# aclyde11/molecular-VAE

Measured on AMD Instinct MI355X. Metric: molecules/s (ELBO fwd+bwd+step), higher is better.
Workload: dtype bf16

## Files before the change

### molecular-vae_amd/csrc/rnn.hip

```cpp
#include "tile_pipe.hpp"
#include "kernels.hpp"
#include <stdlib.h>

template <typename T> __device__ __forceinline__ void load8(const T* p, float (&v)[8]);
template <> __device__ __forceinline__ void load8<float>(const float* p, float (&v)[8]) {
  const float4 a = *reinterpret_cast<const float4*>(p), b = *reinterpret_cast<const float4*>(p + 4);
  v[0] = a.x; v[1] = a.y; v[2] = a.z; v[3] = a.w; v[4] = b.x; v[5] = b.y; v[6] = b.z; v[7] = b.w;
}
template <> __device__ __forceinline__ void load8<bf16_t>(const bf16_t* p, float (&v)[8]) {
  const uint4 u = *reinterpret_cast<const uint4*>(p);
  const uint32_t w[4] = {u.x, u.y, u.z, u.w};
#pragma unroll
  for (int i = 0; i < 4; ++i) { v[2 * i] = __builtin_bit_cast(float, w[i] << 16); v[2 * i + 1] = __builtin_bit_cast(float, w[i] & 0xffff0000u); }
}
template <typename T> __device__ __forceinline__ void store8(T* p, const float (&v)[8]);
template <> __device__ __forceinline__ void store8<float>(float* p, const float (&v)[8]) {
  *reinterpret_cast<float4*>(p) = make_float4(v[0], v[1], v[2], v[3]);
  *reinterpret_cast<float4*>(p + 4) = make_float4(v[4], v[5], v[6], v[7]);
}
template <> __device__ __forceinline__ void store8<bf16_t>(bf16_t* p, const float (&v)[8]) {
  uint4 u;
  u.x = (uint32_t)f2bf(v[0]) | ((uint32_t)f2bf(v[1]) << 16); u.y = (uint32_t)f2bf(v[2]) | ((uint32_t)f2bf(v[3]) << 16);
  u.z = (uint32_t)f2bf(v[4]) | ((uint32_t)f2bf(v[5]) << 16); u.w = (uint32_t)f2bf(v[6]) | ((uint32_t)f2bf(v[7]) << 16);
  *reinterpret_cast<uint4*>(p) = u;
}
template <typename T> __device__ __forceinline__ void ldn(const T* p, float (&v)[8], int n, bool vec) {
  if (vec && n == 8) { load8<T>(p, v); return; }
#pragma unroll
  for (int e = 0; e < 8; ++e) v[e] = (e < n) ? TT<T>::ld(p + e) : 0.f;
}
template <typename T> __device__ __forceinline__ void stn(T* p, const float (&v)[8], int n, bool vec) {
  if (vec && n == 8) { store8<T>(p, v); return; }
#pragma unroll
  for (int e = 0; e < 8; ++e) if (e < n) TT<T>::st(p + e, v[e]);
}

template <typename T> __device__ __forceinline__ float act_sigmoid(float x);
template <typename T> __device__ __forceinline__ float act_tanh(float x);
template <> __device__ __forceinline__ float act_sigmoid<float>(float x) { return 1.f / (1.f + expf(-x)); }
template <> __device__ __forceinline__ float act_tanh<float>(float x) { return tanhf(x); }
template <> __device__ __forceinline__ float act_sigmoid<bf16_t>(float x) { return __builtin_amdgcn_rcpf(1.f + __expf(-x)); }
template <> __device__ __forceinline__ float act_tanh<bf16_t>(float x) { return fmaf(-2.f, __builtin_amdgcn_rcpf(1.f + __expf(2.f * x)), 1.f); }

__device__ __forceinline__ int xcd_remap_r(int bid, int n) {
  const int q = n >> 3, r = n & 7, x = bid & 7, i = bid >> 3;
  return (x < r ? x * (q + 1) : r * (q + 1) + (x - r) * q) + i;
}

struct DropArgs { float scale; uint32_t thresh, seed; };
__host__ __device__ __forceinline__ uint32_t drop_hash(uint32_t seed, uint32_t idx) {
  uint32_t h = idx * 0x9E3779B1u ^ seed;
  h ^= h >> 16; h *= 0x85EBCA6Bu; h ^= h >> 13; h *= 0xC2B2AE35u; h ^= h >> 16;
  return h;
}
__device__ __forceinline__ float drop_factor(const DropArgs& da, const uint8_t* mask, uint32_t idx0, long off) {
  const bool keep = mask ? (mask[off] != 0) : (drop_hash(da.seed, idx0 + (uint32_t)off) >= da.thresh);
  return keep ? da.scale : 0.f;
}

struct StepTaskF {
  const void *A0, *A1, *W0, *W1;
  long lda0, lda1, ldw0, ldw1;
  int K0, K1;
  const float* add; long add_ld;
  const float* add_tbl;
  const int64_t* add_idx; long add_idx_ld; int add_rows;
  const float* bias;
  const float* c_prev; float* c_out;
  void* c_save;
  void* h_out; long ldh;
  void* g_out;
  const void* hprev_t0;
  int t;
  void* h_drop;
  const uint8_t* dmask;
  uint32_t didx0;
};
struct StepArgsF { StepTaskF t[MVAE_MAX_LAYERS]; const int* lengths; int ntask, B, H, tiles_m, tiles_j, dbg, vec, cell, gru3; DropArgs drop; };

template <typename T, int BM, int BJ, int NBUF, bool WS = false>
__global__ __launch_bounds__(WS ? 512 : 256) void lstm_step_fwd_kernel(StepArgsF p) {
  constexpr bool PIPE = NBUF > 0;
  constexpr int NTHR = WS ? 512 : 256;
  static_assert(!WS || NBUF > 0, "wave specialisation needs the LDS-direct ring");
  extern __shared__ __attribute__((aligned(16))) char smem[];
  static_assert(BJ == 32 || BJ == 64, "hidden units per tile");
  constexpr int JS = BJ / 32;
  constexpr int BN = 4 * BJ, WM = BM / 2, MI = WM / 16, NI = 4 * JS;
  const int tid = threadIdx.x, lane = tid & 63, wave = (tid >> 6) & 3, wm = wave >> 1, wj = wave & 1;
  const int per_task = p.tiles_m * p.tiles_j;
  const int bid = xcd_remap_r(blockIdx.x, p.ntask * per_task);
  const int task = bid / per_task;
  const int rem = bid - task * per_task;
  const int tj = rem / p.tiles_m, tm = rem - tj * p.tiles_m;
  const StepTaskF& q = p.t[task];
  const int m0 = tm * BM, j0 = tj * BJ, H = p.H, B = p.B;

  f32x4 acc[MI][NI];
#pragma unroll
  for (int i = 0; i < MI; ++i)
#pragma unroll
    for (int g = 0; g < NI; ++g) acc[i][g] = f32x4{0.f, 0.f, 0.f, 0.f};

#ifdef MVAE_TUNING
  const bool run_main = !(p.dbg & 2);
#else
  constexpr bool run_main = true;
#endif
  if (run_main) {
  if constexpr (PIPE) {
    PipeSeg<BM, BN> s0, s1;
    const uint32_t sz = (uint32_t)sizeof(T);
    const int skip0 = p.gru3 ? 3 : -1, skip1 = p.gru3 ? 2 : -1;
    {
      const uint32_t lda = (uint32_t)q.lda0 * sz, ldw = (uint32_t)q.ldw0 * sz;
      auto offA = [&](int r) -> uint32_t { const int gm = m0 + r; return gm < B ? (uint32_t)gm * lda : PIPE_OOB; };
      auto offB = [&](int r) -> uint32_t { const int g = r / BJ, j = j0 + (r - g * BJ); return (j < H && g != skip0) ? (uint32_t)(g * H + j) * ldw : PIPE_OOB; };
      pipe_seg_init<T, BM, BN>(s0, q.A0, (uint32_t)B * lda, q.W0, (uint32_t)(4 * H) * ldw, offA, offB, q.K0, tid & 255);
    }
    {
      const uint32_t lda = (uint32_t)q.lda1 * sz, ldw = (uint32_t)q.ldw1 * sz;
      auto offA = [&](int r) -> uint32_t { const int gm = m0 + r; return gm < B ? (uint32_t)gm * lda : PIPE_OOB; };
      auto offB = [&](int r) -> uint32_t { const int g = r / BJ, j = j0 + (r - g * BJ); return (j < H && g != skip1) ? (uint32_t)(g * H + j) * ldw : PIPE_OOB; };
      pipe_seg_init<T, BM, BN>(s1, q.A1, (uint32_t)B * lda, q.W1, (uint32_t)(4 * H) * ldw, offA, offB, q.K1, tid & 255);
    }
    if constexpr (WS) tile_gemm_ws<T, BM, BN, MI, NI, (NBUF > 0 ? NBUF : 3), JS, BJ>(smem, s0, s1, wm * WM, wj * (BJ / 2), acc, tid);
    else tile_gemm_pipe<T, BM, BN, MI, NI, (NBUF > 0 ? NBUF : 3), JS, BJ>(smem, s0, s1, wm * WM, wj * (BJ / 2), acc, tid);
  } else {
    int brow[NI];
#pragma unroll
    for (int g = 0; g < NI; ++g) brow[g] = (g / JS) * BJ + wj * (BJ / 2) + (g % JS) * 16;
    if (q.A0 != nullptr) {
      const T* A = reinterpret_cast<const T*>(q.A0);
      const T* W = reinterpret_cast<const T*>(q.W0);
      const long lda = q.lda0, ldw = q.ldw0;
      auto rowA = [&](int r) -> const T* { const int gm = m0 + r; return gm < B ? A + (long)gm * lda : nullptr; };
      auto rowB = [&](int r) -> const T* { const int g = r / BJ, j = j0 + (r - g * BJ); return (j < H && !(p.gru3 && g == 3)) ? W + ((long)g * H + j) * ldw : nullptr; };
      tile_gemm_segment<T, BM, BN, MI, NI>(smem, rowA, rowB, 0, q.K0, wm * WM, brow, acc, tid);
    }
    if (q.A1 != nullptr) {
      const T* A = reinterpret_cast<const T*>(q.A1);
      const T* W = reinterpret_cast<const T*>(q.W1);
      const long lda = q.lda1, ldw = q.ldw1;
      auto rowA = [&](int r) -> const T* { const int gm = m0 + r; return gm < B ? A + (long)gm * lda : nullptr; };
      auto rowB = [&](int r) -> const T* { const int g = r / BJ, j = j0 + (r - g * BJ); return (j < H && !(p.gru3 && g == 2)) ? W + ((long)g * H + j) * ldw : nullptr; };
      tile_gemm_segment<T, BM, BN, MI, NI>(smem, rowA, rowB, 0, q.K1, wm * WM, brow, acc, tid);
    }
// ... 130 lines not shown
        c[e] = gf[e] * cp[e] + gi[e] * gg[e];
        h[e] = go[e] * act_tanh<T>(c[e]);
      }
      st32(q.c_out + (long)row * H + j8, c);
      stT(hout + (long)row * q.ldh + j8, h);
      if (q.h_drop) {
        float hd[8];
#pragma unroll
        for (int e = 0; e < 8; ++e) hd[e] = (e < n) ? h[e] * drop_factor(p.drop, q.dmask, q.didx0, (long)row * H + j8 + e) : 0.f;
        stT(reinterpret_cast<T*>(q.h_drop) + (long)row * q.ldh + j8, hd);
      }
      if (gout) {
        stT(csave + (long)row * H + j8, c);
        stT(g4, gi); stT(g4 + H, gf); stT(g4 + 2 * H, gg); stT(g4 + 3 * H, go);
      }
    } else {
      const bool valid = p.lengths ? (q.t < p.lengths[row]) : true;
      float gr[8], gz[8], gn[8], hs_[8], hseq[8];
#pragma unroll
      for (int e = 0; e < 8; ++e) {
        gr[e] = act_sigmoid<T>(pre[0][e]); gz[e] = act_sigmoid<T>(pre[1][e]);
        gn[e] = act_tanh<T>(pre[2][e] + gr[e] * pre[3][e]);
        const float hn = (1.f - gz[e]) * gn[e] + gz[e] * cp[e];
        hs_[e] = valid ? hn : cp[e];
        hseq[e] = valid ? hn : 0.f;
      }
      st32(q.c_out + (long)row * H + j8, hs_);
      stT(hout + (long)row * q.ldh + j8, hseq);
      if (q.h_drop) {
        float hd[8];
#pragma unroll
        for (int e = 0; e < 8; ++e) hd[e] = (e < n) ? hseq[e] * drop_factor(p.drop, q.dmask, q.didx0, (long)row * H + j8 + e) : 0.f;
        stT(reinterpret_cast<T*>(q.h_drop) + (long)row * q.ldh + j8, hd);
      }
      if (gout) { stT(g4, gr); stT(g4 + H, gz); stT(g4 + 2 * H, gn); stT(g4 + 3 * H, pre[3]); }
    }
  }
  };
  const bool has_add = q.add != nullptr || q.add_tbl != nullptr;
  if (fast) { if (has_add) rows(std::true_type{}, std::true_type{}); else rows(std::true_type{}, std::false_type{}); }
  else { if (has_add) rows(std::false_type{}, std::true_type{}); else rows(std::false_type{}, std::false_type{}); }
}

template <int BMW, int BNB, int NBUF, bool WS = false>
__global__ __launch_bounds__(WS ? 512 : BMW * 2) void lstm_step_fwd_gm_kernel(StepArgsF p) {
  using T = bf16_t;
  extern __shared__ __attribute__((aligned(16))) char smem[];
  static_assert(BMW == 256 || BMW == 128, "weight rows per tile: 64 or 32 units x 4 gates");
  static_assert(!WS || BMW == 128, "loader / consumer split: the 4-wave tile only");
  constexpr int NT = BMW * 2;
  constexpr int BU = BMW / 4;
  constexpr int MI = 8, NI = BNB / 64;
  const int tid = threadIdx.x, lane = tid & 63, wave = WS ? ((tid >> 6) & 3) : (tid >> 6), wm = wave >> 2, wn = wave & 3;
  const int per_task = p.tiles_m * p.tiles_j;
  const int bid = xcd_remap_r(blockIdx.x, p.ntask * per_task);
  const int task = bid / per_task;
  const int rem = bid - task * per_task;
  const int tj = rem / p.tiles_m, tm = rem - tj * p.tiles_m;
  const StepTaskF& q = p.t[task];
  const int n0 = tm * BNB, j0 = tj * BU, H = p.H, B = p.B;

  const int lq = lane >> 4, lc = lane & 15;
  const int ub = j0 + 32 * wm + 8 * lq;
  constexpr bool BIAS_FIRST = (BMW == 256 && BNB == 256);
  auto load_bias = [&](float (&bias)[4][8]) {
    if (q.bias) {
#pragma unroll
      for (int g = 0; g < 4; ++g) load8<float>(q.bias + g * H + ub, bias[g]);
    } else {
#pragma unroll
      for (int g = 0; g < 4; ++g)
#pragma unroll
        for (int e = 0; e < 8; ++e) bias[g][e] = 0.f;
    }
  };
  f32x4 acc[MI][NI];
  if constexpr (BIAS_FIRST) {
    float bias[4][8];
    load_bias(bias);
#pragma unroll
    for (int ni = 0; ni < NI; ++ni)
#pragma unroll
      for (int g = 0; g < 4; ++g)
#pragma unroll
        for (int e = 0; e < 8; ++e) acc[2 * g + (e >> 2)][ni][e & 3] = bias[g][e];
  } else {
#pragma unroll
    for (int i = 0; i < MI; ++i)
#pragma unroll
      for (int g = 0; g < NI; ++g) acc[i][g] = f32x4{0.f, 0.f, 0.f, 0.f};
  }

  float cpa[NI][8];
  auto load_cprev_all = [&]() {
    const float* cpsrc = q.c_prev ? q.c_prev : q.c_out;
#pragma unroll
    for (int ni = 0; ni < NI; ++ni) {
      const int row = n0 + wn * (16 * NI) + ni * 16 + lc;
      load8<float>(cpsrc + (long)(row < B ? row : B - 1) * H + ub, cpa[ni]);
    }
  };
  if constexpr (BIAS_FIRST) load_cprev_all();

#ifdef MVAE_TUNING
  const bool run_main = !(p.dbg & 2);
#else
  constexpr bool run_main = true;
#endif
  if (run_main) {
    PipeSeg<BMW, BNB, NT> s0, s1;
    auto wrow = [&](int r) -> int {
// ... 53 lines not shown
    if constexpr (decltype(has_add)::value) {
#pragma unroll
      for (int g = 0; g < 4; ++g) {
        float a[8];
        load8<float>(q.add + (long)row * q.add_ld + g * H + ub, a);
#pragma unroll
        for (int e = 0; e < 8; ++e) pre[g][e] += a[e];
      }
    }
    float gi[8], gf[8], gg[8], go[8], c[8], h[8];
#pragma unroll
    for (int e = 0; e < 8; ++e) {
      gi[e] = act_sigmoid<T>(pre[0][e]); gf[e] = act_sigmoid<T>(pre[1][e]); gg[e] = act_tanh<T>(pre[2][e]); go[e] = act_sigmoid<T>(pre[3][e]);
      c[e] = gf[e] * cp[e] + gi[e] * gg[e];
      h[e] = go[e] * act_tanh<T>(c[e]);
    }
#ifdef MVAE_TUNING
    const int srow = (p.dbg & 4) ? n0 + (row & 15) : row;
    const bool sgate = !(p.dbg & 8);
#else
    const int srow = row;
    constexpr bool sgate = true;
#endif
    store8<float>(q.c_out + (long)srow * H + ub, c);
    store8<T>(hout + (long)srow * q.ldh + ub, h);
    if (gout) {
      T* g4 = gout + (long)srow * 4 * H + ub;
      store8<T>(csave + (long)srow * H + ub, c);
      if (sgate) { store8<T>(g4, gi); store8<T>(g4 + H, gf); store8<T>(g4 + 2 * H, gg); store8<T>(g4 + 3 * H, go); }
    }
  }
  };
  const bool full = n0 + BNB <= B;
  if (q.add) { if (full) epilogue(std::true_type{}, std::true_type{}); else epilogue(std::true_type{}, std::false_type{}); }
  else { if (full) epilogue(std::false_type{}, std::true_type{}); else epilogue(std::false_type{}, std::false_type{}); }
}

struct StepTaskB {
  const void *A0, *A1, *W0, *W1;
  long lda0, lda1, ldw0, ldw1;
  int K0, K1;
  const float* dy; long dy_ld;
  const void* gates; const void* c; const void* c_prev;
  const float* dc_in; float* dc_out;
  void* dG; long ldg;
  const void* h_prev; long ldhp;
  float* dh0;
  int t;
  int seg1_full;
  int drop;
  const uint8_t* dmask;
  uint32_t didx0;
};
struct StepArgsB { StepTaskB t[MVAE_MAX_LAYERS]; const int* lengths; float* partial; int ntask, B, H, tiles_m, tiles_n, dbg, vec, cell, split, gru3; DropArgs drop; };

template <typename T>
__device__ __forceinline__ void bwd_cell_group(const StepArgsB& p, const StepTaskB& q, int row, int j8, int n, bool vec, float (&dh)[8]) {
  const int H = p.H;
  const T* gates = reinterpret_cast<const T*>(q.gates);
  const T* cs = reinterpret_cast<const T*>(q.c);
  const T* csp = reinterpret_cast<const T*>(q.c_prev);
  T* dG = reinterpret_cast<T*>(q.dG);
  const long o = (long)row * H + j8;
  float dci[8];
  if (q.dc_in) ldn<float>(q.dc_in + o, dci, n, vec);
  else {
#pragma unroll
    for (int e = 0; e < 8; ++e) dci[e] = 0.f;
  }
  if (p.cell == MVAE_CELL_LSTM) {
    if (q.dy) {
      float a[8];
      ldn<float>(q.dy + (long)row * q.dy_ld + j8, a, n, vec);
#pragma unroll
      for (int e = 0; e < 8; ++e) dh[e] += a[e];
    }
    float gi[8], gf[8], gg[8], go[8], c[8], cp[8];
    const T* g4 = gates + (long)row * 4 * H + j8;
    ldn<T>(g4, gi, n, vec); ldn<T>(g4 + H, gf, n, vec); ldn<T>(g4 + 2 * H, gg, n, vec); ldn<T>(g4 + 3 * H, go, n, vec);
    ldn<T>(cs + o, c, n, vec);
    if (csp) ldn<T>(csp + o, cp, n, vec);
    else {
#pragma unroll
      for (int e = 0; e < 8; ++e) cp[e] = 0.f;
    }
    float di[8], df[8], dg[8], dO[8], dco[8];
#pragma unroll
    for (int e = 0; e < 8; ++e) {
      const float tc = act_tanh<T>(c[e]);
      const float d_o = dh[e] * tc;
      const float dc = dh[e] * go[e] * (1.f - tc * tc) + dci[e];
      dco[e] = dc * gf[e];
      di[e] = dc * gg[e] * gi[e] * (1.f - gi[e]);
      df[e] = dc * cp[e] * gf[e] * (1.f - gf[e]);
      dg[e] = dc * gi[e] * (1.f - gg[e] * gg[e]);
      dO[e] = d_o * go[e] * (1.f - go[e]);
    }
    stn<float>(q.dc_out + o, dco, n, vec);
    T* d4 = dG + (long)row * q.ldg + j8;
    stn<T>(d4, di, n, vec); stn<T>(d4 + H, df, n, vec); stn<T>(d4 + 2 * H, dg, n, vec); stn<T>(d4 + 3 * H, dO, n, vec);
  } else {
#pragma unroll
    for (int e = 0; e < 8; ++e) dh[e] += dci[e];
    if (q.gates == nullptr) {
      stn<float>(q.dh0 + o, dh, n, vec);
      return;
    }
// ... 138 lines not shown
template <bool HAS_DY>
__device__ __forceinline__ void bwd_raw_load(const StepArgsB& p, const StepTaskB& q, int row, int j8, BwdRaw& r) {
  const int H = p.H;
  const bf16_t* gates = reinterpret_cast<const bf16_t*>(q.gates);
  const long o = (long)row * H + j8;
  const float* dsrc = (q.dc_in ? q.dc_in : q.dc_out) + o;
  r.dci[0] = *reinterpret_cast<const float4*>(dsrc); r.dci[1] = *reinterpret_cast<const float4*>(dsrc + 4);
  if (gates == nullptr) return;
  if constexpr (HAS_DY) {
    const float* ysrc = q.dy ? q.dy + (long)row * q.dy_ld + j8 : q.dc_out + o;
    r.dy[0] = *reinterpret_cast<const float4*>(ysrc); r.dy[1] = *reinterpret_cast<const float4*>(ysrc + 4);
  }
  const bf16_t* g4 = gates + (long)row * 4 * H + j8;
  r.g[0] = *reinterpret_cast<const uint4*>(g4); r.g[1] = *reinterpret_cast<const uint4*>(g4 + H);
  r.g[2] = *reinterpret_cast<const uint4*>(g4 + 2 * H); r.g[3] = *reinterpret_cast<const uint4*>(g4 + 3 * H);
  if (p.cell == MVAE_CELL_LSTM) {
    const bf16_t* cs = reinterpret_cast<const bf16_t*>(q.c);
    const bf16_t* csp = reinterpret_cast<const bf16_t*>(q.c_prev);
    r.c = *reinterpret_cast<const uint4*>(cs + o);
    r.cp = *reinterpret_cast<const uint4*>((csp ? csp : cs) + o);
  } else {
    r.cp = *reinterpret_cast<const uint4*>(q.h_prev ? reinterpret_cast<const bf16_t*>(q.h_prev) + (long)row * q.ldhp + j8 : g4);
  }
}
__device__ __forceinline__ void unpack8(const uint4& u, float (&v)[8]) {
  const uint32_t w[4] = {u.x, u.y, u.z, u.w};
#pragma unroll
  for (int i = 0; i < 4; ++i) { v[2 * i] = __builtin_bit_cast(float, w[i] << 16); v[2 * i + 1] = __builtin_bit_cast(float, w[i] & 0xffff0000u); }
}
template <bool HAS_DY>
__device__ __forceinline__ void bwd_raw_unpack(const BwdRaw& r, BwdOps& o) {
  o.dci[0] = r.dci[0].x; o.dci[1] = r.dci[0].y; o.dci[2] = r.dci[0].z; o.dci[3] = r.dci[0].w;
  o.dci[4] = r.dci[1].x; o.dci[5] = r.dci[1].y; o.dci[6] = r.dci[1].z; o.dci[7] = r.dci[1].w;
  if constexpr (HAS_DY) {
    o.dy[0] = r.dy[0].x; o.dy[1] = r.dy[0].y; o.dy[2] = r.dy[0].z; o.dy[3] = r.dy[0].w;
    o.dy[4] = r.dy[1].x; o.dy[5] = r.dy[1].y; o.dy[6] = r.dy[1].z; o.dy[7] = r.dy[1].w;
  } else {
#pragma unroll
    for (int e = 0; e < 8; ++e) o.dy[e] = 0.f;
  }
#pragma unroll
  for (int g = 0; g < 4; ++g) unpack8(r.g[g], o.g[g]);
  unpack8(r.c, o.c); unpack8(r.cp, o.cp);
}

template <typename T, int BM, int BN, int NBUF, bool WS = false, bool DROP = false, int SPLITMODE = -1, int PREF = 0>
__global__ __launch_bounds__(WS ? 512 : 256) void lstm_step_bwd_kernel(StepArgsB p) {
  constexpr bool PIPE = NBUF > 0;
  constexpr int NTHR = WS ? 512 : 256;
  static_assert(!WS || NBUF > 0, "wave specialisation needs the LDS-direct ring");
  extern __shared__ __attribute__((aligned(16))) char smem[];
  constexpr int WM = BM / 2, WN = BN / 2, MI = WM / 16, NI = WN / 16;
  const int tid = threadIdx.x, lane = tid & 63, wave = (tid >> 6) & 3, wm = wave >> 1, wn = wave & 1;
  const int per_task = p.tiles_m * p.tiles_n;
  const int nsp = p.split ? p.split : 1;
  const int bid = xcd_remap_r(blockIdx.x, p.ntask * per_task * nsp);
  const int task2 = bid / per_task;
  const int task = task2 / nsp;
  const int sp = task2 - task * nsp;
  const int seg = (nsp == 4) ? (sp >> 1) : sp;
  const int half = (nsp == 4) ? (sp & 1) : 0;
  const int rem = bid - task2 * per_task;
  int tn = rem / p.tiles_m, tm = rem - tn * p.tiles_m;
  if (p.tiles_m >= 16 && (p.tiles_m & 7) == 0 && (p.tiles_n & 3) == 0) {
    const int blk = rem >> 5, in = rem & 31, mb = p.tiles_m >> 3;
    const int tnb = blk / mb, tmb = blk - tnb * mb;
    tn = 4 * tnb + (in >> 3); tm = 8 * tmb + (in & 7);
  }
  const StepTaskB& q = p.t[task];
  const int m0 = tm * BM, n0 = tn * BN, H = p.H, B = p.B;
  if (p.split && (seg == 0 ? q.A0 == nullptr : q.A1 == nullptr)) return;

  f32x4 acc[MI][NI];
#pragma unroll
  for (int i = 0; i < MI; ++i)
#pragma unroll
    for (int n = 0; n < NI; ++n) acc[i][n] = f32x4{0.f, 0.f, 0.f, 0.f};

  if constexpr (PREF != 0) {
    static_assert(WS && NBUF > 0 && SPLITMODE == 0 && !DROP && sizeof(T) == 2, "prefetching form: fused, wave-specialised, bf16");
    constexpr bool HAS_DY = PREF == 1;
    constexpr int SN = BN + 4, GPR = BN / 8, RPI = NTHR / GPR, NIT = BM / RPI;
    static_assert(BM % RPI == 0, "whole row groups per thread");
    PipeSeg<BM, BN> s0, s1;
#ifdef MVAE_TUNING
    const int am0 = (p.dbg & 4) ? 0 : m0, an0 = (p.dbg & 4) ? 0 : n0;
#else
    const int am0 = m0, an0 = n0;
#endif
    {
      const uint32_t lda = (uint32_t)q.lda0 * 2u, ldw = (uint32_t)q.ldw0 * 2u;
      auto offA = [&](int r) -> uint32_t { return (uint32_t)(am0 + r) * lda; };
      auto offB = [&](int r) -> uint32_t { return (uint32_t)(an0 + r) * ldw; };
      pipe_seg_init<T, BM, BN>(s0, q.A0, (uint32_t)B * lda, q.W0, (uint32_t)H * ldw, offA, offB, p.gru3 ? 3 * H : q.K0, tid & 255);
      if (p.gru3) { s0.hole_st = (int)(2 * H * 2 / KB); s0.hole_bytes = (uint32_t)H * 2u; }
    }
    {
      const uint32_t lda = (uint32_t)q.lda1 * 2u, ldw = (uint32_t)q.ldw1 * 2u;
      auto offA = [&](int r) -> uint32_t { return (uint32_t)(am0 + r) * lda; };
      auto offB = [&](int r) -> uint32_t { return (uint32_t)(an0 + r) * ldw; };
      pipe_seg_init<T, BM, BN>(s1, q.A1, (uint32_t)B * lda, q.W1, (uint32_t)H * ldw, offA, offB, (p.gru3 && !q.seg1_full) ? 3 * H : q.K1, tid & 255);
    }
    const int nk = s0.nk + s1.nk;
    const int wv = __builtin_amdgcn_readfirstlane(tid >> 6);
    const int g8 = tid % GPR, j8 = n0 + g8 * 8, row0 = m0 + tid / GPR;
    float* stg = reinterpret_cast<float*>(smem);
    BwdRaw raw[NIT];
    auto finish_all = [&]() {
#pragma unroll
      for (int it = 0; it < NIT; ++it) {
        const int lrow = tid / GPR + it * RPI;
        const float* sp_ = stg + lrow * SN + g8 * 8;
        const float4 a = *reinterpret_cast<const float4*>(sp_), b = *reinterpret_cast<const float4*>(sp_ + 4);
        float dh[8] = {a.x, a.y, a.z, a.w, b.x, b.y, b.z, b.w};
        BwdOps o;
        bwd_raw_unpack<HAS_DY>(raw[it], o);
        bwd_cell_finish<T, true>(p, q, m0 + lrow, j8, 8, true, o, dh);
      }
    };
#ifdef MVAE_TUNING
    const bool run_main = !(p.dbg & 2);
// ... 278 lines not shown
  for (int l = 0; l < NL; ++l) drop = drop || d->hdrop[l] != nullptr;
  if (drop) {
    if (!(d->drop_p > 0.f) || d->drop_p >= 1.f) return MVAE_ERR_INVALID;
    for (int l = 0; l + 1 < NL; ++l) if (!d->hdrop[l]) return MVAE_ERR_INVALID;
  }
  if (!drop) {
    const int rc = rnn_rowres_fwd(d, st);
    if (rc != MVAE_ERR_UNSUPPORTED) return rc;
  }
  if (!drop) {
    const int rc = rnn_gru_rowres_fwd(d, st);
    if (rc != MVAE_ERR_UNSUPPORTED) return rc;
  }
  auto nblk = [&](int bm) { return (long)((B + bm - 1) / bm) * ((H + 31) / 32) * NL; };
  int BM = (nblk(128) >= 256) ? 128 : (nblk(64) >= 256 || dt == MVAE_BF16) ? 64 : 32;
  if (dt == MVAE_BF16) BM = 64;
  BM = tune_int("MVAE_BM", BM);
  if (BM == 32 && dt == MVAE_BF16) BM = 64;
  const int sz = (dt == MVAE_BF16) ? 2 : 4, ke = KB / sz;
  int Hk = H;
  if (d->zero_padded_k && H % ke) {
    const int hp = (H + ke - 1) / ke * ke;
    bool ok = d->ldh >= hp && (!d->h0[0] || d->ldh0 >= hp);
    for (int l = 0; l < NL; ++l) ok = ok && d->ldw_hh[l] >= hp && (l == 0 || d->ldw_ih[l] >= hp);
    if (ok) Hk = hp;
  }
  bool pipe = (Hk % ke == 0) && (d->ldh % (16 / sz) == 0) && ((long)B * d->ldh * sz < (1L << 31)) && (!d->x0 || (d->in0 % ke == 0 && d->x0_ld % (16 / sz) == 0)) &&
              (!d->h0[0] || d->ldh0 % (16 / sz) == 0);
  bool vec = (H % 8 == 0) && (d->ldh % 8 == 0) && (!d->add0 || (al16(d->add0) && d->add0_tstride % 4 == 0)) && (!d->add_table || al16(d->add_table));
  for (int l = 0; l < NL; ++l) {
    if ((4L * H) * d->ldw_hh[l] * sz >= (1L << 31) || d->ldw_hh[l] % (16 / sz)) pipe = false;
    if ((l > 0 || d->x0) && ((4L * H) * d->ldw_ih[l] * sz >= (1L << 31) || d->ldw_ih[l] % (16 / sz))) pipe = false;
    if (!al16(d->hs[l]) || (!gru && !infer && !al16(d->cs[l])) || (!infer && !al16(d->gates[l])) || !al16(d->cstate[l]) || (d->bias[l] && !al16(d->bias[l]))) vec = false;
    if (d->h0[l] && (!al16(d->h0[l]) || d->ldh0 % 8)) vec = false;
  }
  StepArgsF a;
  a.lengths = d->lengths; a.cell = d->cell;
  int BJ = (pipe && dt == MVAE_BF16 && (long)((B + 127) / 128) * ((H + 63) / 64) * NL >= 256) ? 64 : 32;
  BJ = tune_int("MVAE_BJ", BJ);
  if (BJ == 64 && (!pipe || dt != MVAE_BF16)) BJ = 32;
  if (BJ == 64) BM = 128;
  const int gm_knob = tune_int("MVAE_FWD_GM", 1);
  int BMW = 0, BNB = 0;
  for (int l = 0; l < NL && drop; ++l) if (d->hdrop[l] && (!al16(d->hdrop[l]))) vec = false;
  if (gm_knob && !gru && !drop && !d->add_table && dt == MVAE_BF16 && pipe && vec && H % 64 == 0) {
    static const int cand[4][2] = {{256, 256}, {256, 128}, {128, 128}, {128, 64}};
    for (int c = 0; c < 4 && !BMW; ++c) {
      const long tiles = (long)((B + cand[c][1] - 1) / cand[c][1]) * (H / (cand[c][0] / 4)) * NL;
      const bool chosen = gm_knob == 1 && tiles >= 192 && ((c == 0 && B >= 256) || (c == 3 && B >= 64 && B <= 128));
      if (gm_knob == cand[c][0] * 1000 + cand[c][1] || chosen) { BMW = cand[c][0]; BNB = cand[c][1]; }
    }
  }
  if (BMW) { BM = BNB; BJ = BMW / 4; }
  a.B = B; a.H = H; a.tiles_m = (B + BM - 1) / BM; a.tiles_j = (H + BJ - 1) / BJ; a.vec = vec ? 1 : 0;
  a.drop.scale = drop ? 1.f / (1.f - d->drop_p) : 1.f;
  a.drop.thresh = drop ? (uint32_t)((double)d->drop_p * 4294967296.0) : 0u;
  a.drop.seed = d->drop_seed;
  a.gru3 = gru ? 1 : 0;
#ifdef MVAE_TUNING
  a.dbg = tune_int("MVAE_DBG", 0);
#else
  a.dbg = 0;
#endif
  int nbuf_dflt = (BJ == 64) ? 3 : (dt == MVAE_BF16 && BM == 64) ? 3 : 4;
  if (dt == MVAE_BF16 && BM == 64 && BJ == 32 && !BMW) {
    const long nb = (long)((B + BM - 1) / BM) * ((H + BJ - 1) / BJ) * NL, cus = 256;
    if ((nb + 3 * cus - 1) / (3 * cus) < (nb + 2 * cus - 1) / (2 * cus)) nbuf_dflt = 2;
  }
  const int nbuf = pipe ? tune_int("MVAE_NBUF_FWD", nbuf_dflt) : 0;
  size_t lds = (size_t)(nbuf > 0 ? nbuf : 2) * (BM + 4 * BJ) * KB;
  const size_t stage_bytes = (size_t)BM * 4 * (BJ + 4) * sizeof(float);
  if (lds < stage_bytes) lds = stage_bytes;
  for (int dd = 0; dd < T + NL - 1; ++dd) {
    int n = 0;
    for (int l = 0; l < NL; ++l) {
      const int t = dd - l;
      if (t < 0 || t >= T) continue;
      StepTaskF& q = a.t[n++];
      if (l == 0) {
        q.A0 = d->x0 ? adv(d->x0, (long)t * B * d->x0_ld, dt) : nullptr;
        q.lda0 = d->x0_ld; q.K0 = d->in0; q.W0 = d->w_ih[0]; q.ldw0 = d->ldw_ih[0];
        q.add = d->add0 ? d->add0 + (long)t * d->add0_tstride : nullptr;
        q.add_ld = 4L * H;
        q.add_tbl = d->add_table; q.add_idx = d->add_table ? d->add_index + t : nullptr; q.add_idx_ld = d->add_index_ld; q.add_rows = d->add_table_rows;
      } else {
        q.A0 = adv(drop ? d->hdrop[l - 1] : d->hs[l - 1], (long)t * B * d->ldh, dt);
        q.lda0 = d->ldh; q.K0 = Hk; q.W0 = d->w_ih[l]; q.ldw0 = d->ldw_ih[l];
        q.add = nullptr; q.add_ld = 0;
        q.add_tbl = nullptr; q.add_idx = nullptr; q.add_idx_ld = 0; q.add_rows = 0;
      }
      q.A1 = (t > 0) ? adv(d->hs[l], (long)(t - 1) * B * d->ldh, dt) : d->h0[l];
      q.lda1 = (t > 0) ? d->ldh : d->ldh0;
      q.K1 = Hk; q.W1 = d->w_hh[l]; q.ldw1 = d->ldw_hh[l];
      q.bias = d->bias[l];
      q.c_prev = (t > 0) ? d->cstate[l] + (long)((t - 1) & 1) * B * H : nullptr;
      q.c_out = d->cstate[l] + (long)(t & 1) * B * H;
      q.c_save = (gru || infer) ? nullptr : const_cast<char*>(adv(d->cs[l], (long)t * B * H, dt));
      q.hprev_t0 = (gru && t == 0) ? d->h0[l] : nullptr;
      q.t = t;
      q.h_drop = (drop && l + 1 < NL) ? const_cast<char*>(adv(d->hdrop[l], (long)t * B * d->ldh, dt)) : nullptr;
      q.dmask = (drop && d->drop_mask[l]) ? d->drop_mask[l] + ((long)t * B) * H : nullptr;
      q.didx0 = (uint32_t)((((long)l * T + t) * B) * H);
      q.h_out = const_cast<char*>(adv(d->hs[l], (long)t * B * d->ldh, dt)); q.ldh = d->ldh;
      q.g_out = infer ? nullptr : const_cast<char*>(adv(d->gates[l], (long)t * B * 4 * H, dt));
    }
    a.ntask = n;
    dim3 grid(n * a.tiles_m * a.tiles_j), block(256);
    if (BMW) {
      block = dim3(BMW * 2);
      if (BMW == 256 && BNB == 256) {
        lds = 2 * (256 + 256) * KB;
        MVAE_STEP_LAUNCH((lstm_step_fwd_gm_kernel<256, 256, 2>));
      }
      else if (BMW == 256) { lds = 3 * (256 + 128) * KB; MVAE_STEP_LAUNCH((lstm_step_fwd_gm_kernel<256, 128, 3>)); }
      else if (BNB == 128) { lds = 4 * (128 + 128) * KB; MVAE_STEP_LAUNCH((lstm_step_fwd_gm_kernel<128, 128, 4>)); }
      else { lds = 4 * (128 + 64) * KB; block = dim3(512); MVAE_STEP_LAUNCH((lstm_step_fwd_gm_kernel<128, 64, 4, true>)); }
      continue;
    }
#define FWD_CASE(TT_, BM_, NB_) if (BJ == 32 && BM == BM_ && nbuf == NB_) { MVAE_STEP_LAUNCH((lstm_step_fwd_kernel<TT_, BM_, 32, NB_>)); continue; }
    if (BJ == 64 && nbuf == 3) {
      block = dim3(512); MVAE_STEP_LAUNCH((lstm_step_fwd_kernel<bf16_t, 128, 64, 3, true>));
      continue;
    }
    if (dt == MVAE_BF16) {
      FWD_CASE(bf16_t, 128, 0) FWD_CASE(bf16_t, 128, 3) FWD_CASE(bf16_t, 128, 4) FWD_CASE(bf16_t, 128, 5)
      FWD_CASE(bf16_t, 64, 0) FWD_CASE(bf16_t, 64, 2) FWD_CASE(bf16_t, 64, 3) FWD_CASE(bf16_t, 64, 4) FWD_CASE(bf16_t, 64, 5)
    } else {
      FWD_CASE(float, 128, 0) FWD_CASE(float, 128, 4) FWD_CASE(float, 64, 0) FWD_CASE(float, 64, 4) FWD_CASE(float, 32, 0) FWD_CASE(float, 32, 4)
    }
#undef FWD_CASE
    return MVAE_ERR_UNSUPPORTED;
  }
  MVAE_CHECK_HIP(hipGetLastError());
  return MVAE_OK;
}

int rnn_rowres_bwd(const mvae_rnn_bwd_desc* d, hipStream_t st);
int rnn_gru_rowres_bwd(const mvae_rnn_bwd_desc* d, hipStream_t st);
size_t rnn_rowres_bwd_workspace(int layers, int T, int B, int H);

size_t rnn_bwd_workspace_bytes(const mvae_rnn_bwd_desc* d) {
  if (!d || d->layers < 1 || d->B < 1 || d->H < 1 || d->T < 1) return 0;
  const size_t split = (size_t)d->layers * 4 * d->B * d->H * sizeof(float);
  const size_t rowres = rnn_rowres_bwd_workspace(d->layers, d->T, d->B, d->H);
  return split > rowres ? split : rowres;
}

int rnn_bwd_impl(const mvae_rnn_bwd_desc* d, hipStream_t st) {
  if (!d) return MVAE_ERR_INVALID;
  if (d->cell != MVAE_CELL_LSTM && d->cell != MVAE_CELL_GRU) return MVAE_ERR_UNSUPPORTED;
  if (d->layers < 1 || d->layers > MVAE_MAX_LAYERS || d->T < 1 || d->B < 1 || d->H < 1) return MVAE_ERR_INVALID;
  if (d->dtype != MVAE_F32 && d->dtype != MVAE_BF16) return MVAE_ERR_INVALID;
  const int NL = d->layers, T = d->T, B = d->B, H = d->H, dt = d->dtype;
  const int epc = (dt == MVAE_BF16) ? 8 : 4;
  const bool gru = d->cell == MVAE_CELL_GRU;
  if (!d->dy && !d->dy_a && !gru) return MVAE_ERR_INVALID;
  if (d->dy_a && (!d->dy_w || d->dy_k < 128 || d->dy_k % 128 || d->dy_a_ld < d->dy_k || d->dy_w_ld < d->dy_k || d->dy_a_ld % epc || d->dy_w_ld % epc ||
                  ((reinterpret_cast<uintptr_t>(d->dy_a) | reinterpret_cast<uintptr_t>(d->dy_w)) & 15)))
    return MVAE_ERR_INVALID;
  if (d->lengths && !gru) return MVAE_ERR_UNSUPPORTED;
  for (int l = 0; l < NL && !gru; ++l)
    if (d->h0[l] || d->dh_last[l] || d->dh0[l]) return MVAE_ERR_UNSUPPORTED;
  for (int l = 0; l < NL; ++l) {
    if (!d->w_hhT[l] || (!gru && !d->cs[l]) || !d->gates[l] || !d->dG[l] || !d->dstate[l]) return MVAE_ERR_INVALID;
    if (gru && !d->hs[l]) return MVAE_ERR_INVALID;
    if (l > 0 && !d->w_ihT[l]) return MVAE_ERR_INVALID;
    if (d->ldw_hhT[l] % epc || (l > 0 && d->ldw_ihT[l] % epc)) return MVAE_ERR_INVALID;
  }
  const long ldg = d->ldg;
  if (ldg < 4L * H || ldg % epc) return MVAE_ERR_INVALID;
  const bool drop = d->drop_p > 0.f;
  if (drop && d->drop_p >= 1.f) return MVAE_ERR_INVALID;
  if (!drop) {
    const int rc = rnn_rowres_bwd(d, st);
    if (rc != MVAE_ERR_UNSUPPORTED) return rc;
  }
  if (!drop) {
    const int rc = rnn_gru_rowres_bwd(d, st);
    if (rc != MVAE_ERR_UNSUPPORTED) return rc;
  }
  int BM = 64, BN = 64;
  if (dt == MVAE_F32 && (long)((B + 63) / 64) * ((H + 63) / 64) * NL < 256) { BM = 32; BN = 32; }
  if (!drop) BM = tune_int("MVAE_BM", BM);
  if (BM == 32 && dt == MVAE_BF16) BM = 64;
  if (BM != 32) BN = 64;
  const int sz = (dt == MVAE_BF16) ? 2 : 4, ke = KB / sz;
  bool pipe = ((4 * H) % ke == 0) && ((long)B * ldg * sz < (1L << 31)) && (ldg % (16 / sz) == 0);
  bool vec = (H % 8 == 0) && (ldg % 8 == 0) && (!d->dy || (al16(d->dy) && (d->dy_ld % 4 == 0)));
  for (int l = 0; l < NL; ++l) {
    if ((long)H * d->ldw_hhT[l] * sz >= (1L << 31) || d->ldw_hhT[l] % (16 / sz)) pipe = false;
    if (l > 0 && ((long)H * d->ldw_ihT[l] * sz >= (1L << 31) || d->ldw_ihT[l] % (16 / sz))) pipe = false;
    if ((!gru && !al16(d->cs[l])) || !al16(d->gates[l]) || !al16(d->dG[l]) || !al16(d->dstate[l])) vec = false;
    if (gru && (!al16(d->hs[l]) || d->ldh % 8 || (d->h0[l] && (!al16(d->h0[l]) || d->ldh0 % 8)))) vec = false;
    if (d->dh_last[l] && !al16(d->dh_last[l])) vec = false;
    if (d->dh0[l] && !al16(d->dh0[l])) vec = false;
  }
  if (d->dy_a && (!pipe || dt != MVAE_BF16 || (long)B * d->dy_a_ld * sz >= (1L << 31) || (long)H * d->dy_w_ld * sz >= (1L << 31))) return MVAE_ERR_UNSUPPORTED;
  const int split_knob = tune_int("MVAE_BWD_SPLIT", 1);
  int nsplit = 0;
  if (split_knob && dt == MVAE_BF16 && pipe && vec && B % 128 == 0 && H % 128 == 0 && d->split_ws) {
    struct Cand { int bm, bn, ns, key; };
    static const Cand cand[7] = {{256, 128, 1, 2561}, {128, 128, 1, 1281}, {128, 64, 1, 641}, {256, 128, 2, 2562}, {128, 128, 2, 2}, {128, 128, 4, 1284}, {128, 64, 4, 644}};
    for (int c = 0; c < 7 && !nsplit; ++c) {
      if (B % cand[c].bm || (cand[c].ns == 4 && (4 * H) % (2 * ke))) continue;
      if (drop && cand[c].ns == 1) continue;
      const long wgs = (long)(B / cand[c].bm) * (H / cand[c].bn) * cand[c].ns * NL;
      if (split_knob == cand[c].key || (split_knob == 1 && wgs >= (cand[c].ns == 1 ? 256 : 192))) { BM = cand[c].bm; BN = cand[c].bn; nsplit = cand[c].ns; }
    }
    if (!nsplit && split_knob == 1 && (4 * H) % (2 * ke) == 0 && (long)(B / 128) * (H / 64) * 4 * NL >= 64) { BM = 128; BN = 64; nsplit = 4; }
    if (nsplit > 1 && d->split_ws_bytes < (size_t)NL * nsplit * B * H * sizeof(float)) { nsplit = 0; BM = 64; BN = 64; }
    if (split_knob == 1 && nsplit > 1) {
      const long fused_tiles = (long)((B + 63) / 64) * ((H + 63) / 64) * NL;
      const long kcols = (gru ? 6L : 8L) * H;
      if (fused_tiles >= 192 && 128 * kcols * sz <= (1L << 20)) { nsplit = 0; BM = 64; BN = 64; }
      if (NL == 1 && 128 * kcols * sz <= (1L << 20)) { nsplit = 0; BM = 64; BN = 64; }
    }
  }
  const bool big_fused = nsplit == 1;
  if (big_fused) nsplit = 0;
  const bool split = nsplit != 0;
  StepArgsB a;
  a.lengths = d->lengths; a.cell = d->cell; a.split = nsplit; a.partial = split ? reinterpret_cast<float*>(d->split_ws) : nullptr;
  a.drop.scale = drop ? 1.f / (1.f - d->drop_p) : 1.f;
  a.drop.thresh = drop ? (uint32_t)((double)d->drop_p * 4294967296.0) : 0u;
  a.drop.seed = d->drop_seed;
  a.gru3 = (gru && H % ke == 0 && (nsplit != 4 || (3 * H / 2) % ke == 0)) ? 1 : 0;
  a.B = B; a.H = H; a.tiles_m = (B + BM - 1) / BM; a.tiles_n = (H + BN - 1) / BN; a.vec = vec ? 1 : 0;
#ifdef MVAE_TUNING
  a.dbg = tune_int("MVAE_DBG", 0);
#else
  a.dbg = 0;
#endif
  const int nbuf = pipe ? (drop ? 4 : tune_int("MVAE_NBUF_BWD", 4)) : 0;
  size_t lds = (size_t)(split ? (BM == 256 ? 3 : 4) : big_fused ? (BM == 256 ? 3 : 4) : (nbuf > 0 ? nbuf : 2)) * (BM + BN) * KB;
  const size_t stage_bytes = (size_t)BM * (BN + 4) * sizeof(float);
  if (lds < stage_bytes) lds = stage_bytes;
  bool want_dh0 = false;
  for (int l = 0; l < NL; ++l) want_dh0 = want_dh0 || (gru && d->dh0[l]);
  for (int e = T + NL - 2; e >= (want_dh0 ? -1 : 0); --e) {
    int n = 0;
    if (e < 0) {
      for (int l = 0; l < NL; ++l) {
        if (!d->dh0[l]) continue;
        StepTaskB& q = a.t[n++];
        q.A0 = d->dG[l]; q.lda0 = ldg; q.K0 = 4 * H; q.W0 = d->w_hhT[l]; q.ldw0 = d->ldw_hhT[l];
        q.A1 = nullptr; q.lda1 = ldg; q.K1 = 4 * H; q.W1 = nullptr; q.ldw1 = 0;
        q.dy = nullptr; q.dy_ld = 0; q.gates = nullptr; q.c = nullptr; q.c_prev = nullptr;
        q.dc_in = d->dstate[l]; q.dc_out = nullptr; q.dG = nullptr; q.ldg = ldg; q.h_prev = nullptr; q.ldhp = 0;
        q.dh0 = d->dh0[l]; q.t = -1; q.drop = 0; q.dmask = nullptr; q.didx0 = 0; q.seg1_full = 0;
      }
      if (n == 0) break;
    }
    for (int l = 0; l < NL && e >= 0; ++l) {
      const int t = e - l;
      if (t < 0 || t >= T) continue;
      StepTaskB& q = a.t[n++];
      q.A0 = (t < T - 1) ? adv(d->dG[l], (long)(t + 1) * B * ldg, dt) : nullptr;
      q.lda0 = ldg; q.K0 = 4 * H; q.W0 = d->w_hhT[l]; q.ldw0 = d->ldw_hhT[l];
      q.A1 = (l < NL - 1) ? adv(d->dG[l + 1], (long)t * B * ldg, dt) : nullptr;
      q.lda1 = ldg; q.K1 = 4 * H; q.W1 = (l < NL - 1) ? d->w_ihT[l + 1] : nullptr; q.ldw1 = (l < NL - 1) ? d->ldw_ihT[l + 1] : 0;
      q.seg1_full = 0;
      if (l == NL - 1 && d->dy_a) {
        q.A1 = adv(d->dy_a, (long)t * B * d->dy_a_ld, dt); q.lda1 = d->dy_a_ld; q.K1 = d->dy_k; q.W1 = d->dy_w; q.ldw1 = d->dy_w_ld;
        q.seg1_full = 1;
      }
      q.dy = (l == NL - 1 && d->dy) ? d->dy + (long)t * B * d->dy_ld : nullptr; q.dy_ld = d->dy_ld;
      q.gates = adv(d->gates[l], (long)t * B * 4 * H, dt);
      q.c = gru ? nullptr : adv(d->cs[l], (long)t * B * H, dt);
      q.c_prev = (!gru && t > 0) ? adv(d->cs[l], (long)(t - 1) * B * H, dt) : nullptr;
      q.dc_in = (t < T - 1) ? d->dstate[l] + (long)((t + 1) & 1) * B * H : (gru ? d->dh_last[l] : nullptr);
      q.h_prev = gru ? ((t > 0) ? adv(d->hs[l], (long)(t - 1) * B * d->ldh, dt) : d->h0[l]) : nullptr;
      q.ldhp = (t > 0) ? d->ldh : d->ldh0;
      q.dh0 = nullptr; q.t = t;
      q.drop = (drop && l < NL - 1) ? 1 : 0;
      q.dmask = (q.drop && d->drop_mask[l]) ? d->drop_mask[l] + ((long)t * B) * H : nullptr;
      q.didx0 = (uint32_t)((((long)l * T + t) * B) * H);
      q.dc_out = d->dstate[l] + (long)(t & 1) * B * H;
      q.dG = const_cast<char*>(adv(d->dG[l], (long)t * B * ldg, dt)); q.ldg = ldg;
    }
    a.ntask = n;
    dim3 grid(n * a.tiles_m * a.tiles_n * (split ? nsplit : 1)), block(256);
    if (big_fused && drop) return MVAE_ERR_UNSUPPORTED;
    if (big_fused) {
      block = dim3(512);
      if (BM == 256) {
        MVAE_STEP_LAUNCH((lstm_step_bwd_kernel<bf16_t, 256, 128, 3, true, false, 0>));
        continue;
      }
      if (BN == 64) {
        if (d->dy) MVAE_STEP_LAUNCH((lstm_step_bwd_kernel<bf16_t, 128, 64, 4, true, false, 0, 1>));
        else MVAE_STEP_LAUNCH((lstm_step_bwd_kernel<bf16_t, 128, 64, 4, true, false, 0, 2>));
        continue;
      }
      if (d->dy) MVAE_STEP_LAUNCH((lstm_step_bwd_kernel<bf16_t, 128, 128, 4, true, false, 0, 1>));
      else MVAE_STEP_LAUNCH((lstm_step_bwd_kernel<bf16_t, 128, 128, 4, true, false, 0, 2>));
      continue;
    }
    if (split) {
      if (BM == 256) { block = dim3(512); MVAE_STEP_LAUNCH((lstm_step_bwd_kernel<bf16_t, 256, 128, 3, true, false, 1>)); block = dim3(256); }
      else if (BN == 64) { block = dim3(512); MVAE_STEP_LAUNCH((lstm_step_bwd_kernel<bf16_t, 128, 64, 4, true, false, 1>)); block = dim3(256); }
      else { block = dim3(512); MVAE_STEP_LAUNCH((lstm_step_bwd_kernel<bf16_t, 128, 128, 4, true, false, 1>)); block = dim3(256); }
      const long groups = (long)n * B * (H / 8);
      hipLaunchKernelGGL((lstm_bwd_epi_kernel<bf16_t>), dim3((unsigned)((groups + 255) / 256)), block, 0, st, a);
      continue;
    }
#define BWD_DROP(TT_, BM_, NB_) if (BM == BM_ && nbuf == NB_) { MVAE_STEP_LAUNCH((lstm_step_bwd_kernel<TT_, BM_, (BM_ == 32 ? 32 : 64), NB_, false, true>)); continue; }
    if (drop) {
      if (dt == MVAE_BF16) { BWD_DROP(bf16_t, 64, 4) BWD_DROP(bf16_t, 64, 0) }
      else { BWD_DROP(float, 64, 4) BWD_DROP(float, 64, 0) BWD_DROP(float, 32, 4) BWD_DROP(float, 32, 0) }
      return MVAE_ERR_UNSUPPORTED;
    }
#undef BWD_DROP
#define BWD_CASE(TT_, BM_, NB_) if (BM == BM_ && nbuf == NB_) { MVAE_STEP_LAUNCH((lstm_step_bwd_kernel<TT_, BM_, (BM_ == 32 ? 32 : 64), NB_>)); continue; }
    if (dt == MVAE_BF16) {
      BWD_CASE(bf16_t, 128, 0) BWD_CASE(bf16_t, 128, 3) BWD_CASE(bf16_t, 128, 4) BWD_CASE(bf16_t, 128, 5) BWD_CASE(bf16_t, 128, 6)
      BWD_CASE(bf16_t, 64, 0) BWD_CASE(bf16_t, 64, 3) BWD_CASE(bf16_t, 64, 4) BWD_CASE(bf16_t, 64, 5) BWD_CASE(bf16_t, 64, 6)
    } else {
      BWD_CASE(float, 128, 0) BWD_CASE(float, 128, 4) BWD_CASE(float, 64, 0) BWD_CASE(float, 64, 4) BWD_CASE(float, 32, 0) BWD_CASE(float, 32, 4)
    }
#undef BWD_CASE
    return MVAE_ERR_UNSUPPORTED;
  }
  MVAE_CHECK_HIP(hipGetLastError());
  return MVAE_OK;
}
```

Measured before the change: 36590.

## Balance tile order across XCDs and use half tiles on diagonal wavefront steps

Moves the XCD block remap into a shared tile_order helper with an optional 'balanced' ordering that interleaves tasks (layers) across groups, so each XCD gets work from every concurrent layer rather than one. It also adds 'half tile' selection on partially filled wavefront diagonals (fewer layers active than NL): the forward GM kernel drops to 128-column tiles and the backward fused kernel to 64-column tiles when the grid would otherwise be small, to raise CU occupancy. The balanced order is on by default in forward for grids of 256 blocks or fewer, and off in backward. Smaller tiles add more weight reloads and per-block overhead.

```diff
diff --git a/molecular-vae_amd/csrc/rnn.hip b/molecular-vae_amd/csrc/rnn.hip
--- a/molecular-vae_amd/csrc/rnn.hip
+++ b/molecular-vae_amd/csrc/rnn.hip
@@ -1,4 +1,5 @@
 #include "tile_pipe.hpp"
+#include "tile_order.hpp"
 #include "kernels.hpp"
 #include <stdlib.h>
 
@@ -41,11 +42,6 @@
 template <> __device__ __forceinline__ float act_tanh<float>(float x) { return tanhf(x); }
 template <> __device__ __forceinline__ float act_sigmoid<bf16_t>(float x) { return __builtin_amdgcn_rcpf(1.f + __expf(-x)); }
 template <> __device__ __forceinline__ float act_tanh<bf16_t>(float x) { return fmaf(-2.f, __builtin_amdgcn_rcpf(1.f + __expf(2.f * x)), 1.f); }
-
-__device__ __forceinline__ int xcd_remap_r(int bid, int n) {
-  const int q = n >> 3, r = n & 7, x = bid & 7, i = bid >> 3;
-  return (x < r ? x * (q + 1) : r * (q + 1) + (x - r) * q) + i;
-}
 
 struct DropArgs { float scale; uint32_t thresh, seed; };
 __host__ __device__ __forceinline__ uint32_t drop_hash(uint32_t seed, uint32_t idx) {
@@ -76,7 +72,7 @@
   const uint8_t* dmask;
   uint32_t didx0;
 };
-struct StepArgsF { StepTaskF t[MVAE_MAX_LAYERS]; const int* lengths; int ntask, B, H, tiles_m, tiles_j, dbg, vec, cell, gru3; DropArgs drop; };
+struct StepArgsF { StepTaskF t[MVAE_MAX_LAYERS]; const int* lengths; int ntask, B, H, tiles_m, tiles_j, dbg, vec, cell, gru3, order; DropArgs drop; };
 
 template <typename T, int BM, int BJ, int NBUF, bool WS = false>
 __global__ __launch_bounds__(WS ? 512 : 256) void lstm_step_fwd_kernel(StepArgsF p) {
@@ -88,11 +84,8 @@
   constexpr int JS = BJ / 32;
   constexpr int BN = 4 * BJ, WM = BM / 2, MI = WM / 16, NI = 4 * JS;
   const int tid = threadIdx.x, lane = tid & 63, wave = (tid >> 6) & 3, wm = wave >> 1, wj = wave & 1;
-  const int per_task = p.tiles_m * p.tiles_j;
-  const int bid = xcd_remap_r(blockIdx.x, p.ntask * per_task);
-  const int task = bid / per_task;
-  const int rem = bid - task * per_task;
-  const int tj = rem / p.tiles_m, tm = rem - tj * p.tiles_m;
+  const TileId ord = tile_order(blockIdx.x, p.ntask, 1, p.tiles_m, p.tiles_j, p.order != 0);
+  const int task = ord.task, tj = ord.tn, tm = ord.tm;
   const StepTaskF& q = p.t[task];
   const int m0 = tm * BM, j0 = tj * BJ, H = p.H, B = p.B;
 
@@ -329,11 +322,8 @@
   constexpr int BU = BMW / 4;
   constexpr int MI = 8, NI = BNB / 64;
   const int tid = threadIdx.x, lane = tid & 63, wave = WS ? ((tid >> 6) & 3) : (tid >> 6), wm = wave >> 2, wn = wave & 3;
-  const int per_task = p.tiles_m * p.tiles_j;
-  const int bid = xcd_remap_r(blockIdx.x, p.ntask * per_task);
-  const int task = bid / per_task;
-  const int rem = bid - task * per_task;
-  const int tj = rem / p.tiles_m, tm = rem - tj * p.tiles_m;
+  const TileId ord = tile_order(blockIdx.x, p.ntask, 1, p.tiles_m, p.tiles_j, p.order != 0);
+  const int task = ord.task, tj = ord.tn, tm = ord.tm;
   const StepTaskF& q = p.t[task];
   const int n0 = tm * BNB, j0 = tj * BU, H = p.H, B = p.B;
 
@@ -493,7 +483,7 @@
   const uint8_t* dmask;
   uint32_t didx0;
 };
-struct StepArgsB { StepTaskB t[MVAE_MAX_LAYERS]; const int* lengths; float* partial; int ntask, B, H, tiles_m, tiles_n, dbg, vec, cell, split, gru3; DropArgs drop; };
+struct StepArgsB { StepTaskB t[MVAE_MAX_LAYERS]; const int* lengths; float* partial; int ntask, B, H, tiles_m, tiles_n, dbg, vec, cell, split, gru3, order; DropArgs drop; };
 
 template <typename T>
 __device__ __forceinline__ void bwd_cell_group(const StepArgsB& p, const StepTaskB& q, int row, int j8, int n, bool vec, float (&dh)[8]) {
@@ -738,21 +728,11 @@
   extern __shared__ __attribute__((aligned(16))) char smem[];
   constexpr int WM = BM / 2, WN = BN / 2, MI = WM / 16, NI = WN / 16;
   const int tid = threadIdx.x, lane = tid & 63, wave = (tid >> 6) & 3, wm = wave >> 1, wn = wave & 1;
-  const int per_task = p.tiles_m * p.tiles_n;
   const int nsp = p.split ? p.split : 1;
-  const int bid = xcd_remap_r(blockIdx.x, p.ntask * per_task * nsp);
-  const int task2 = bid / per_task;
-  const int task = task2 / nsp;
-  const int sp = task2 - task * nsp;
+  const TileId ord = tile_order(blockIdx.x, p.ntask, nsp, p.tiles_m, p.tiles_n, p.order != 0);
+  const int task = ord.task, sp = ord.sp, tn = ord.tn, tm = ord.tm;
   const int seg = (nsp == 4) ? (sp >> 1) : sp;
   const int half = (nsp == 4) ? (sp & 1) : 0;
-  const int rem = bid - task2 * per_task;
-  int tn = rem / p.tiles_m, tm = rem - tn * p.tiles_m;
-  if (p.tiles_m >= 16 && (p.tiles_m & 7) == 0 && (p.tiles_n & 3) == 0) {
-    const int blk = rem >> 5, in = rem & 31, mb = p.tiles_m >> 3;
-    const int tnb = blk / mb, tmb = blk - tnb * mb;
-    tn = 4 * tnb + (in >> 3); tm = 8 * tmb + (in & 7);
-  }
   const StepTaskB& q = p.t[task];
   const int m0 = tm * BM, n0 = tn * BN, H = p.H, B = p.B;
   if (p.split && (seg == 0 ? q.A0 == nullptr : q.A1 == nullptr)) return;
@@ -1137,6 +1117,9 @@
     }
   }
   if (BMW) { BM = BNB; BJ = BMW / 4; }
+  const int order_knob = tune_int("MVAE_XCD_ORDER", -1);
+  const bool diag_tiles = tune_int("MVAE_DIAG_TILES", 1) != 0 && BMW == 256 && BNB == 256;
+  const int full_cells = NL < T ? NL : T;
   a.B = B; a.H = H; a.tiles_m = (B + BM - 1) / BM; a.tiles_j = (H + BJ - 1) / BJ; a.vec = vec ? 1 : 0;
   a.drop.scale = drop ? 1.f / (1.f - d->drop_p) : 1.f;
   a.drop.thresh = drop ? (uint32_t)((double)d->drop_p * 4294967296.0) : 0u;
@@ -1191,14 +1174,20 @@
     }
     a.ntask = n;
     dim3 grid(n * a.tiles_m * a.tiles_j), block(256);
+    a.order = order_knob >= 0 ? order_knob : (grid.x <= 256 ? 1 : 0);
     if (BMW) {
       block = dim3(BMW * 2);
-      if (BMW == 256 && BNB == 256) {
+      const bool half_tile = diag_tiles && n < full_cells && (long)n * ((B + 127) / 128) * a.tiles_j <= 256;
+      const int bnb = half_tile ? 128 : BNB;
+      a.tiles_m = (B + bnb - 1) / bnb;
+      grid = dim3(n * a.tiles_m * a.tiles_j);
+      a.order = order_knob >= 0 ? order_knob : (grid.x <= 256 ? 1 : 0);
+      if (BMW == 256 && bnb == 256) {
         lds = 2 * (256 + 256) * KB;
         MVAE_STEP_LAUNCH((lstm_step_fwd_gm_kernel<256, 256, 2>));
       }
       else if (BMW == 256) { lds = 3 * (256 + 128) * KB; MVAE_STEP_LAUNCH((lstm_step_fwd_gm_kernel<256, 128, 3>)); }
-      else if (BNB == 128) { lds = 4 * (128 + 128) * KB; MVAE_STEP_LAUNCH((lstm_step_fwd_gm_kernel<128, 128, 4>)); }
+      else if (bnb == 128) { lds = 4 * (128 + 128) * KB; MVAE_STEP_LAUNCH((lstm_step_fwd_gm_kernel<128, 128, 4>)); }
       else { lds = 4 * (128 + 64) * KB; block = dim3(512); MVAE_STEP_LAUNCH((lstm_step_fwd_gm_kernel<128, 64, 4, true>)); }
       continue;
     }
@@ -1304,7 +1293,10 @@
   const bool big_fused = nsplit == 1;
   if (big_fused) nsplit = 0;
   const bool split = nsplit != 0;
+  const bool diag_tiles = tune_int("MVAE_DIAG_TILES", 1) != 0 && big_fused && BM == 128 && BN == 128;
+  const int full_cells = NL < T ? NL : T;
   StepArgsB a;
+  a.order = tune_int("MVAE_XCD_ORDER", 0);
   a.lengths = d->lengths; a.cell = d->cell; a.split = nsplit; a.partial = split ? reinterpret_cast<float*>(d->split_ws) : nullptr;
   a.drop.scale = drop ? 1.f / (1.f - d->drop_p) : 1.f;
   a.drop.thresh = drop ? (uint32_t)((double)d->drop_p * 4294967296.0) : 0u;
@@ -1317,9 +1309,11 @@
   a.dbg = 0;
 #endif
   const int nbuf = pipe ? (drop ? 4 : tune_int("MVAE_NBUF_BWD", 4)) : 0;
-  size_t lds = (size_t)(split ? (BM == 256 ? 3 : 4) : big_fused ? (BM == 256 ? 3 : 4) : (nbuf > 0 ? nbuf : 2)) * (BM + BN) * KB;
-  const size_t stage_bytes = (size_t)BM * (BN + 4) * sizeof(float);
-  if (lds < stage_bytes) lds = stage_bytes;
+  auto lds_bytes = [&](int bn) {
+    const size_t ring = (size_t)(split ? (BM == 256 ? 3 : 4) : big_fused ? (BM == 256 ? 3 : 4) : (nbuf > 0 ? nbuf : 2)) * (BM + bn) * KB;
+    const size_t stage_bytes = (size_t)BM * (bn + 4) * sizeof(float);
+    return ring < stage_bytes ? stage_bytes : ring;
+  };
   bool want_dh0 = false;
   for (int l = 0; l < NL; ++l) want_dh0 = want_dh0 || (gru && d->dh0[l]);
   for (int e = T + NL - 2; e >= (want_dh0 ? -1 : 0); --e) {
@@ -1364,6 +1358,10 @@
       q.dG = const_cast<char*>(adv(d->dG[l], (long)t * B * ldg, dt)); q.ldg = ldg;
     }
     a.ntask = n;
+    const bool half_tile = diag_tiles && e >= 0 && n < full_cells && (long)n * a.tiles_m * (H / 64) <= 256;
+    const int bn = half_tile ? 64 : BN;
+    a.tiles_n = (H + bn - 1) / bn;
+    const size_t lds = lds_bytes(bn);
     dim3 grid(n * a.tiles_m * a.tiles_n * (split ? nsplit : 1)), block(256);
     if (big_fused && drop) return MVAE_ERR_UNSUPPORTED;
     if (big_fused) {
@@ -1372,7 +1370,7 @@
         MVAE_STEP_LAUNCH((lstm_step_bwd_kernel<bf16_t, 256, 128, 3, true, false, 0>));
         continue;
       }
-      if (BN == 64) {
+      if (bn == 64) {
         if (d->dy) MVAE_STEP_LAUNCH((lstm_step_bwd_kernel<bf16_t, 128, 64, 4, true, false, 0, 1>));
         else MVAE_STEP_LAUNCH((lstm_step_bwd_kernel<bf16_t, 128, 64, 4, true, false, 0, 2>));
         continue;
diff --git a/molecular-vae_amd/csrc/tile_order.hpp b/molecular-vae_amd/csrc/tile_order.hpp
--- /dev/null
+++ b/molecular-vae_amd/csrc/tile_order.hpp
@@ -0,0 +1,36 @@
+#pragma once
+
+#if defined(__HIPCC__) || defined(__CUDACC__)
+#define TILE_ORDER_FN __host__ __device__ __forceinline__
+#else
+#define TILE_ORDER_FN static inline
+#endif
+
+TILE_ORDER_FN int xcd_remap_r(int bid, int n) {
+  const int q = n >> 3, r = n & 7, x = bid & 7, i = bid >> 3;
+  return (x < r ? x * (q + 1) : r * (q + 1) + (x - r) * q) + i;
+}
+
+TILE_ORDER_FN bool tile_order_blocked(int tiles_m, int tiles_n) { return tiles_m >= 16 && (tiles_m & 7) == 0 && (tiles_n & 3) == 0; }
+TILE_ORDER_FN int tile_order_group(int tiles_m, int tiles_n) { return tile_order_blocked(tiles_m, tiles_n) ? 32 : tiles_m; }
+
+struct TileId { int task, sp, tm, tn; };
+
+TILE_ORDER_FN TileId tile_order(int bid, int ntask, int nsp, int tiles_m, int tiles_n, bool balanced) {
+  const int per_part = tiles_m * tiles_n, nparts = ntask * nsp;
+  const bool blocked = tile_order_blocked(tiles_m, tiles_n);
+  const int gsz = blocked ? 32 : tiles_m, gpp = per_part / gsz;
+  const int v = xcd_remap_r(bid, nparts * per_part);
+  const int s = v / gsz, in = v - s * gsz;
+  const int d = balanced ? nparts : gpp, hi = s / d, lo = s - hi * d;
+  const int part = balanced ? lo : hi, grp = balanced ? hi : lo;
+  TileId r;
+  r.task = part / nsp; r.sp = part - r.task * nsp;
+  if (blocked) {
+    const int mb = tiles_m >> 3, tnb = grp / mb, tmb = grp - tnb * mb;
+    r.tn = 4 * tnb + (in >> 3); r.tm = 8 * tmb + (in & 7);
+  } else {
+    r.tn = grp; r.tm = in;
+  }
+  return r;
+}
```

Result: no change. 36700 (median of 6 runs) (+0.3%).
